# amikey/kaldi-ctc

Measured on AMD Instinct MI355X. Metric: CTC-train frames/sec, 5×BLSTM-512 mb=16, at 1/2/4/8 MI355X; loss match, higher is better.
Workload: dtype f32

## Files before the change

### kaldi-ctc_amd/_bindings.py

```python
import ctypes

vp, ci, cl, cf, cd, sz = (ctypes.c_void_p, ctypes.c_int, ctypes.c_long, ctypes.c_float,
                          ctypes.c_double, ctypes.c_size_t)
ip = ctypes.POINTER(ctypes.c_int)

SIGS = {
    "krnnCreate": (ci, [ctypes.POINTER(vp), ci, ci, ci, ci, ci]),
    "krnnDestroy": (ci, [vp]),
    "krnnGetStatusString": (ctypes.c_char_p, [ci]),
    "krnnGetParamsSize": (sz, [vp]),
    "krnnGetLinLayerOffset": (cl, [vp, ci, ci, ci, ip]),
    "krnnGetWorkspaceSize": (sz, [vp, ci, ci]),
    "krnnGetTrainingReserveSize": (sz, [vp, ci, ci]),
    "krnnForwardTraining": (ci, [vp, vp, ci, ci, vp, vp, vp, vp, sz, vp, sz]),
    "krnnForwardInference": (ci, [vp, vp, ci, ci, vp, vp, vp, vp, sz]),
    "krnnGetInferenceSeqWorkspaceSize": (sz, [vp, ci, ci]),
    "krnnForwardInferenceSeq": (ci, [vp, vp, ci, ci, vp, vp, vp, vp, vp, sz]),
    "krnnBackwardData": (ci, [vp, vp, ci, ci, vp, vp, vp, vp, vp, sz, vp, sz]),
    "krnnBackwardWeights": (ci, [vp, vp, ci, ci, vp, vp, vp, sz, vp, vp, sz]),
    "krnnGetDeviceStatus": (ci, [vp, vp]),
    "kcm_add_mat_mat": (ci, [vp, ci, ci, ci, ci, ci, cf, vp, cl, vp, cl, cf, vp, cl]),
    "kcm_add_mat_mat_x3_workspace": (sz, [ci, ci, ci]),
    "kcm_add_mat_mat_x3": (ci, [vp, ci, ci, ci, ci, ci, cf, vp, cl, vp, cl, cf, vp, cl, vp]),
    "kcm_bench_gemm_packed": (cf, [vp, ci, ci, ci, ci, ci, ci]),
    "kcm_test_gemm_packed": (ci, [vp, ci, ci, ci, ci, ci, ci, ci, ci, vp, vp, vp, vp]),
    "kcm_test_row_stream": (ci, [vp, ci, ci, ci, ci, ci, vp, vp, vp, vp]),
    "kctc_test_component_side_streams": (ci, [vp, ci]),
    "kctc_test_rec6_select": (ci, [ci, ci, ci, ci, ci, ci, ip, ctypes.POINTER(vp)]),
    "kctc_test_rec_plan": (ci, [ci, ci, ci, ci, ci, ci, ctypes.POINTER(cl)]),
    "kcm_find_row_max_id": (ci, [vp, vp, cl, ci, vp]),
    "kcm_clip_gradient_rows": (ci, [vp, vp, cl, ci, cf, vp]),
    "kcm_add_vec_clipped": (ci, [vp, vp, vp, cl, cf, cf]),
    "kcm_add_row_sum_mat": (ci, [vp, vp, cl, ci, cf, cf, vp, vp]),
    "kctc_last_error": (ctypes.c_char_p, []),
    "kctc_nnet_create": (ci, [ctypes.POINTER(vp), ctypes.c_char_p, ctypes.c_ulonglong, ci]),
    "kctc_nnet_destroy": (ci, [vp]),
    "kctc_nnet_num_components": (ci, [vp]),
    "kctc_nnet_context": (ci, [vp, ip, ip]),
    "kctc_nnet_component_info": (ci, [vp, ci, ctypes.c_char_p, sz]),
    "kctc_nnet_num_params": (cl, [vp, ci]),
    "kctc_nnet_get_params": (ci, [vp, ci, vp, cl]),
    "kctc_nnet_set_params": (ci, [vp, ci, vp, cl]),
    "kctc_nnet_get_grad": (ci, [vp, ci, vp, cl]),
    "kctc_nnet_set_learning_rate": (ci, [vp, cf]),
    "kctc_nnet_clip_stats": (ci, [vp, ci, ctypes.POINTER(cd), ctypes.POINTER(cd)]),
    "kctc_nnet_srand": (ci, [vp, ctypes.c_uint]),
    "kctc_nnet_rand_calls": (ci, [vp, ctypes.POINTER(cl)]),
    "kctc_nnet_last_best_path": (ci, [vp, vp, cl]),
    "kctc_nnet_last_output": (ci, [vp, vp, cl]),
    "kctc_nnet_last_costs": (ci, [vp, vp, ci]),
    "kctc_nnet_train_step": (ci, [vp, vp, ci, ci, vp, vp, vp, ctypes.POINTER(cd), ctypes.POINTER(cd),
                                  ctypes.POINTER(cd)]),
# ... 108 lines not shown
```

### kaldi-ctc_amd/csrc/ctc.hip

```cpp
#include <algorithm>
#include <cstring>
#include <type_traits>
#include <atomic>
#include <vector>

#include "common.h"
#include "ctc.h"
#include "prof.h"

namespace kctc {
namespace ctcimpl {

constexpr int kMaxLabel = 639;
constexpr int kThreads = 256;
constexpr int kABThreads = 512;
constexpr int kABWaves = kABThreads / 64;
constexpr int kSPT = (2 * kMaxLabel + 1 + kABThreads - 1) / kABThreads;
constexpr int kFR = 8;

struct UttDesc {
  int T, L, S, feasible, lab_off, pad;
  long long ab_off;
  long long off_off;
};

struct Layout {
  size_t desc, labels, links, owner, costs, logz, lp, spill, offs, total;
  int T_max;
  long long spill_floats, off_doubles;
};
// ... 464 lines not shown

template <bool SPILL>
__global__ __launch_bounds__(64 * kWinWaves) void ctc_alpha_beta_win(
    const float *__restrict__ lp, int N, int A, int blank, UttDesc *__restrict__ descs,
    const int *__restrict__ labels, float *__restrict__ spill, double *__restrict__ offs,
    double *__restrict__ costs, AbLds lay) {
  if (blockIdx.x >= (unsigned)N) win_body<SPILL, true>(lp, N, A, blank, descs, labels, spill, offs, costs, lay);
  else win_body<SPILL, false>(lp, N, A, blank, descs, labels, spill, offs, costs, lay);
}

template <bool SPILL, int SPT>
__global__ __launch_bounds__(kABThreads) void ctc_alpha_beta(
    const float *__restrict__ lp, int N, int A, int blank, UttDesc *__restrict__ descs,
    const int *__restrict__ labels, float *__restrict__ spill, double *__restrict__ offs,
    double *__restrict__ costs, AbLds lay) {
  if (blockIdx.x >= (unsigned)N) ab_body<SPILL, SPT, true>(lp, N, A, blank, descs, labels, spill, offs, costs, lay);
  else ab_body<SPILL, SPT, false>(lp, N, A, blank, descs, labels, spill, offs, costs, lay);
}

__global__ __launch_bounds__(kThreads) void ctc_grad(
    const float *__restrict__ acts, const float *__restrict__ logz, float *__restrict__ grads,
    int N, int A, int T_max, int blank, const UttDesc *__restrict__ descs,
    const int *__restrict__ links, const int *__restrict__ owners, const float *__restrict__ spill,
    const double *__restrict__ offs, const double *__restrict__ costs) {
  extern __shared__ __attribute__((aligned(16))) char smem[];
  const int n = blockIdx.y, t0 = blockIdx.x * kFR, tid = threadIdx.x;
  const UttDesc d = descs[n];
  const int T = d.feasible ? d.T : 0, L = d.L, S = d.S;
  const int nf = min(kFR, T_max - t0);
  if (t0 >= T) {
    for (int it = tid; it < nf * A; it += kThreads) {
      int f = it / A, a = it - f * A;
      grads[((long)(t0 + f) * N + n) * A + a] = 0.f;
    }
    return;
  }
  float *occ = reinterpret_cast<float *>(smem);
  int *nxt = reinterpret_cast<int *>(occ + kFR * S);
  int *owner = nxt + (L > 0 ? L : 1);
  float *gblank = reinterpret_cast<float *>(owner + A);
  float *gtot = gblank + kFR;
  for (int a = tid; a < A; a += kThreads) owner[a] = owners[(long)n * A + a];
  for (int j = tid; j < L; j += kThreads) nxt[j] = links[d.lab_off + j];
  const double logp = -costs[n];
  const float *al = spill + d.ab_off;
  const float *be = al + (long long)T * S;
  const double *oa = offs + d.off_off, *ob = oa + T;
  const int nreal = min(nf, T - t0);
  for (int f = 0; f < nreal; f++) {
    const int t = t0 + f;
    const float Kt = (float)(oa[t] + ob[t] - logp);
    for (int s = tid; s < S; s += kThreads) {
      float v = al[(long)t * S + s] + be[(long)t * S + s];
      occ[f * S + s] = (v == -INFINITY) ? 0.f : expf(v + Kt);
    }
  }
// ... 6 lines not shown
        acc += occ[f * S + s];
        tot += occ[f * S + s] + (s + 1 < S ? occ[f * S + s + 1] : 0.f);
      }
      acc = wave_sum(acc);
      tot = wave_sum(tot);
      if (lane == 0) { gblank[f] = acc / tot; gtot[f] = 1.f / tot; }
    }
  }
  __syncthreads();
  for (int it = tid; it < nf * A; it += kThreads) {
    const int f = it / A, a = it - f * A, t = t0 + f;
    const long idx = ((long)t * N + n) * A + a;
    float g = 0.f;
    if (t < T) {
      float gam = 0.f;
      if (a == blank) {
        gam = gblank[f];
      } else {
        for (int j = owner[a]; j >= 0; j = nxt[j]) gam += occ[f * S + 2 * j + 1];
        gam *= gtot[f];
      }
      g = expf(acts[idx] - logz[(long)t * N + n]) - gam;
    }
    grads[idx] = g;
  }
}

struct Staging {
  char *buf = nullptr;
  size_t cap = 0;
  hipEvent_t ev = nullptr;
  bool pending = false;
};
static thread_local Staging g_stage;

static char *staging_acquire(size_t bytes) {
  Staging &s = g_stage;
  if (s.pending) {
    if (hipEventSynchronize(s.ev) != hipSuccess) return nullptr;
    s.pending = false;
  }
  if (!s.ev && hipEventCreateWithFlags(&s.ev, hipEventDisableTiming) != hipSuccess) return nullptr;
  if (bytes > s.cap) {
    if (s.buf) (void)hipHostFree(s.buf);
    size_t cap = align_up(bytes * 2, 4096);
    if (hipHostMalloc((void **)&s.buf, cap, hipHostMallocDefault) != hipSuccess) {
      s.buf = nullptr; s.cap = 0;
// ... 4 lines not shown
  return s.buf;
}
static void staging_release(hipStream_t stream) {
  if (hipEventRecord(g_stage.ev, stream) == hipSuccess) g_stage.pending = true;
}

static std::atomic<int> g_frame_group{0};
static int frame_group() {
  int m = g_frame_group.load(std::memory_order_relaxed);
  if (m <= 0) {
    m = 8;
    int expect = 0;
    g_frame_group.compare_exchange_strong(expect, m);
    m = g_frame_group.load(std::memory_order_relaxed);
  }
  return m;
}

static std::atomic<int> g_win{1};
static bool win_enabled() { return g_win.load(std::memory_order_relaxed) != 0; }

static ctcStatus_t launch(const float *acts, float *grads, const int *flat_labels,
                          const int *label_lengths, const int *input_lengths, int A, int N,
                          double *costs_dev, void *workspace, hipStream_t stream, int blank) {
  Layout lay;
  std::vector<UttDesc> descs;
  bool bad = false;
  if (!make_layout(label_lengths, input_lengths, A, N, &lay, &descs, &bad) || bad)
    return CTC_STATUS_INVALID_VALUE;
  if (blank < 0 || blank >= A || !acts || !workspace) return CTC_STATUS_INVALID_VALUE;
  long long nlab = 0;
  for (int n = 0; n < N; n++) nlab += label_lengths[n];
  for (long long i = 0; i < nlab; i++)
    if (flat_labels[i] < 0 || flat_labels[i] >= A || flat_labels[i] == blank)
      return CTC_STATUS_INVALID_VALUE;
  char *ws = static_cast<char *>(workspace);
  char *stage = staging_acquire(lay.costs);
  if (!stage) return CTC_STATUS_MEMOPS_FAILED;
  memcpy(stage + lay.desc, descs.data(), sizeof(UttDesc) * N);
  if (nlab) memcpy(stage + lay.labels, flat_labels, sizeof(int) * nlab);
  {
    int *links = reinterpret_cast<int *>(stage + lay.links), *owner = reinterpret_cast<int *>(stage + lay.owner);
    std::fill(owner, owner + (size_t)N * A, -1);
    long long off = 0;
    for (int n = 0; n < N; n++) {
      const int L = label_lengths[n];
      int *own = owner + (size_t)n * A;
// ... 52 lines not shown
        hipLaunchKernelGGL(kern, dim3(grid), dim3(kABThreads), shm, stream, d_lp, N, A, blank, d_desc, d_lab,
                           d_spill, d_offs, costs_dev, al);
      };
      if (Smax <= kABThreads) {
        if (want) go(ctc_alpha_beta<true, 1>, 2 * N);
        else go(ctc_alpha_beta<false, 1>, N);
      } else {
        if (want) go(ctc_alpha_beta<true, kSPT>, 2 * N);
        else go(ctc_alpha_beta<false, kSPT>, N);
      }
    }
  }
  if (want && lay.T_max > 0) {
    int Lmax = 0;
    for (int n = 0; n < N; n++) Lmax = label_lengths[n] > Lmax ? label_lengths[n] : Lmax;
    const int Smax = 2 * Lmax + 1;
    size_t shm = sizeof(float) * kFR * Smax + sizeof(int) * (Lmax > 0 ? Lmax : 1) +
                 sizeof(int) * A + 2 * sizeof(float) * kFR;
    if (shm > 160 * 1024) return CTC_STATUS_INVALID_VALUE;
    ProfSpan ps(stream, "ctc_grad");
    hipLaunchKernelGGL(ctc_grad, dim3(ceil_div(lay.T_max, kFR), N), dim3(kThreads), shm, stream,
                       acts, d_logz, grads, N, A, lay.T_max, blank, d_desc,
                       reinterpret_cast<const int *>(ws + lay.links), reinterpret_cast<const int *>(ws + lay.owner),
                       d_spill, d_offs, costs_dev);
  }
  if (hipGetLastError() != hipSuccess) return CTC_STATUS_EXECUTION_FAILED;
  return CTC_STATUS_SUCCESS;
}

}
}

using namespace kctc::ctcimpl;

extern "C" {

int get_warpctc_version(void) { return 2; }

int mictc_set_frame_group(int m) {
  const int prev = frame_group();
  if (m > 0) g_frame_group.store(std::max(1, std::min(m, 8)));
  return prev;
}

int mictc_set_win(int on) {
  const int prev = g_win.load();
  if (on >= 0) g_win.store(on ? 1 : 0);
// ... 4 lines not shown
  switch (status) {
    case CTC_STATUS_SUCCESS: return "no error";
    case CTC_STATUS_MEMOPS_FAILED: return "cuda memcpy or memset failed";
    case CTC_STATUS_INVALID_VALUE: return "invalid value";
    case CTC_STATUS_EXECUTION_FAILED: return "execution failed";
    case CTC_STATUS_UNKNOWN_ERROR:
    default: return "unknown error";
  }
}

ctcStatus_t get_workspace_size(const int *const label_lengths, const int *const input_lengths,
                               int alphabet_size, int minibatch, struct ctcOptions info,
                               size_t *size_bytes) {
  if (!size_bytes || info.loc != CTC_GPU) return CTC_STATUS_INVALID_VALUE;
  Layout lay;
  bool bad = false;
  if (!make_layout(label_lengths, input_lengths, alphabet_size, minibatch, &lay, nullptr, &bad) ||
      bad)
    return CTC_STATUS_INVALID_VALUE;
  *size_bytes = lay.total;
  return CTC_STATUS_SUCCESS;
}

ctcStatus_t mictc_compute_ctc_loss_async(const float *activations, float *gradients,
                                         const int *flat_labels, const int *label_lengths,
                                         const int *input_lengths, int alphabet_size,
                                         int minibatch, double *costs_dev, void *workspace,
                                         ctcStream_t stream, int blank_label) {
  if (!costs_dev) return CTC_STATUS_INVALID_VALUE;
  try {
    return launch(activations, gradients, flat_labels, label_lengths, input_lengths,
                  alphabet_size, minibatch, costs_dev, workspace,
                  reinterpret_cast<hipStream_t>(stream), blank_label);
  } catch (...) {
    return CTC_STATUS_UNKNOWN_ERROR;
  }
}

ctcStatus_t compute_ctc_loss(const float *const activations, float *gradients,
                             const int *const flat_labels, const int *const label_lengths,
                             const int *const input_lengths, int alphabet_size, int minibatch,
                             float *costs, void *workspace, struct ctcOptions options) {
  if (options.loc != CTC_GPU || !costs) return CTC_STATUS_INVALID_VALUE;
  Layout lay;
  bool bad = false;
  if (!make_layout(label_lengths, input_lengths, alphabet_size, minibatch, &lay, nullptr, &bad) ||
      bad)
    return CTC_STATUS_INVALID_VALUE;
  hipStream_t stream = reinterpret_cast<hipStream_t>(options.stream);
  double *d_costs = reinterpret_cast<double *>(static_cast<char *>(workspace) + lay.costs);
  ctcStatus_t st = mictc_compute_ctc_loss_async(activations, gradients, flat_labels,
                                                label_lengths, input_lengths, alphabet_size,
                                                minibatch, d_costs, workspace, options.stream,
                                                options.blank_label);
  if (st != CTC_STATUS_SUCCESS) return st;
  std::vector<double> hc(minibatch);
  if (hipMemcpyAsync(hc.data(), d_costs, sizeof(double) * minibatch, hipMemcpyDeviceToHost,
                     stream) != hipSuccess)
    return CTC_STATUS_MEMOPS_FAILED;
// ... 7 lines not shown
```

### kaldi-ctc_amd/csrc/elementwise.hip

```cpp
#include "common.h"
#include "elementwise.h"

namespace kctc {
namespace {

typedef float floatx4 __attribute__((ext_vector_type(4)));

__global__ __launch_bounds__(256) void k_clip_sgd(float *__restrict__ w, const float *__restrict__ dw,
                                                  long n, float lr, float clip, const unsigned *skip) {
  if (skip && *skip) return;
  const long n4 = n / 4;
  const long stride = (long)gridDim.x * 256;
  const bool vec = ((uintptr_t)w % 16 == 0) && ((uintptr_t)dw % 16 == 0);
  long i = (long)blockIdx.x * 256 + threadIdx.x;
  if (vec) {
    for (; i < n4; i += stride) {
      floatx4 g = reinterpret_cast<const floatx4 *>(dw)[i];
      floatx4 v = reinterpret_cast<floatx4 *>(w)[i];
#pragma unroll
      for (int j = 0; j < 4; j++) {
        float x = g[j];
        if (clip > 0.f) x = fminf(fmaxf(x, -clip), clip);
        v[j] += lr * x;
      }
// ... 65 lines not shown
      const float x = r[j];
      if (x > v[k]) { v[k] = x; vi[k] = j; }
    }
  }
  if (v[2] > v[0]) { v[0] = v[2]; vi[0] = vi[2]; }
  if (v[3] > v[1]) { v[1] = v[3]; vi[1] = vi[3]; }
  if (v[1] > v[0]) { v[0] = v[1]; vi[0] = vi[1]; }
  float b = v[0];
  int bi = vi[0];
#pragma unroll
  for (int w = 32; w >= 1; w >>= 1) {
    const float ob = __shfl_down(b, w, 64);
    const int oi = __shfl_down(bi, w, 64);
    if (ob > b) { b = ob; bi = oi; }
  }
  if (lane == 0) ids[row] = bi;
}

__global__ __launch_bounds__(256) void k_sum_rows(const float *__restrict__ X, long rows, int cols,
                                                  float alpha, float beta, float *__restrict__ out) {
  __shared__ float part[16][64];
  const int c = blockIdx.x * 64 + (threadIdx.x & 63), g = threadIdx.x >> 6;
  float s = 0.f;
  if (c < cols)
    for (long r = blockIdx.y * 4 + g; r < rows; r += 4L * gridDim.y) s += X[r * cols + c];
  part[g][threadIdx.x & 63] = s;
  __syncthreads();
  if (g == 0 && c < cols) {
    float v = ((part[0][threadIdx.x] + part[1][threadIdx.x]) + part[2][threadIdx.x]) + part[3][threadIdx.x];
    out[(long)blockIdx.y * cols + c] = v;
  }
}

__global__ __launch_bounds__(256) void k_sum_partials(const float *__restrict__ part, int nparts,
                                                      int cols, float alpha, float beta,
                                                      float *__restrict__ out) {
  const int c = blockIdx.x * 256 + threadIdx.x;
  if (c >= cols) return;
  float s = 0.f;
  for (int p = 0; p < nparts; p++) s += part[(long)p * cols + c];
  out[c] = alpha * s + (beta != 0.f ? beta * out[c] : 0.f);
}

__global__ void k_scale(float *p, long n, float a) {
  for (long i = (long)blockIdx.x * 256 + threadIdx.x; i < n; i += (long)gridDim.x * 256) p[i] *= a;
}

__global__ void k_fill(float *p, long n, float v) {
  for (long i = (long)blockIdx.x * 256 + threadIdx.x; i < n; i += (long)gridDim.x * 256) p[i] = v;
}

}

static int grid_for(long n, int per = 256) {
  long b = (n + per - 1) / per;
  return (int)std::max<long>(1, std::min<long>(b, 4096));
}

__global__ __launch_bounds__(256) void k_momentum(float *__restrict__ w, float *__restrict__ delta,
                                                  const float *__restrict__ dw, long n, float lr, float clip,
                                                  float m, const unsigned *skip) {
  if (skip && *skip) return;
  for (long i = (long)blockIdx.x * 256 + threadIdx.x; i < n; i += (long)gridDim.x * 256) {
// ... 232 lines not shown
```

### kaldi-ctc_amd/csrc/gemm.h

```cpp
#pragma once
#include <hip/hip_runtime.h>

namespace kctc {

struct GemmArgs {
  bool transA = false, transB = false;
  int M = 0, N = 0, K = 0;
  float alpha = 1.f, beta = 0.f;
  const float *A = nullptr, *B = nullptr;
  float *C = nullptr;
  long lda = 0, ldb = 0, ldc = 0;
  const float *bias = nullptr, *bias2 = nullptr;
  int batch = 1;
  long strideA = 0, strideB = 0, strideC = 0, strideBias = 0;
  int split_k = 1;
  float *ws = nullptr;
  int max_blocks = 0;
  int *tile_counter = nullptr;
};

void gemm_f32(hipStream_t stream, const GemmArgs &g);
int gemm_pick_split(int M, int N, int K, int batch);

void absmax_f32(hipStream_t stream, const float *X, long ldx, int rows, int cols, unsigned *rmax, unsigned *cmax,
                int batch = 1, long strideX = 0, long strideR = 0, long strideC = 0);

void colsum_f32(hipStream_t stream, const float *X, long ldx, int rows, int cols, float alpha,
                float beta, float *out, int batch = 1, long strideX = 0, long strideOut = 0);

}
```

### kaldi-ctc_amd/csrc/gemm.hip

```cpp
#include "common.h"
#include "gemm.h"

namespace kctc {
namespace {

constexpr int BM = 128, BN = 128, BK = 32, LDK = BK + 4, NT = 256;
constexpr int LDM = BM + 4;
constexpr int OPSZ = (BM * LDK > BK * LDM) ? BM * LDK : BK * LDM;
typedef float floatx4 __attribute__((ext_vector_type(4)));

struct KParams {
  const float *A, *B;
  float *C;
  const float *bias, *bias2;
  long lda, ldb, ldc;
  long strideA, strideB, strideC, strideBias;
  int M, N, K, gx, tiles, batch, split, kchunk;
  float alpha, beta;
  float *ws;
  int vecA, vecB;
  int *counter;
};

template <bool KC>
__device__ __forceinline__ void load_tile(const float *__restrict__ P, long ld, int rows, int r0,
                                          int k0, int kend, int vec, floatx4 (&reg)[4]) {
  const int t = threadIdx.x;
#pragma unroll
  for (int i = 0; i < 4; i++) {
    int r, k;
    if (KC) { r = r0 + (t >> 3) + 32 * i; k = k0 + (t & 7) * 4; }
    else    { k = k0 + (t >> 5) + 8 * i;  r = r0 + (t & 31) * 4; }
    floatx4 v = {0.f, 0.f, 0.f, 0.f};
    if (KC) {
      if (r < rows) {
        const float *p = P + (long)r * ld + k;
        if (vec && k + 3 < kend) {
          v = *reinterpret_cast<const floatx4 *>(p);
        } else {
#pragma unroll
          for (int j = 0; j < 4; j++) v[j] = (k + j < kend) ? p[j] : 0.f;
        }
      }
    } else {
      if (k < kend) {
        const float *p = P + (long)k * ld + r;
        if (vec && r + 3 < rows) {
          v = *reinterpret_cast<const floatx4 *>(p);
        } else {
#pragma unroll
          for (int j = 0; j < 4; j++) v[j] = (r + j < rows) ? p[j] : 0.f;
        }
      }
    }
    reg[i] = v;
  }
}

template <bool KC>
__device__ __forceinline__ void store_tile(float *__restrict__ S, const floatx4 (&reg)[4]) {
  const int t = threadIdx.x;
#pragma unroll
  for (int i = 0; i < 4; i++) {
    if (KC) {
      int r = (t >> 3) + 32 * i, k = (t & 7) * 4;
      *reinterpret_cast<floatx4 *>(S + r * LDK + k) = reg[i];
    } else {
      int k = (t >> 5) + 8 * i, r = (t & 31) * 4;
      *reinterpret_cast<floatx4 *>(S + k * LDM + r) = reg[i];
    }
  }
}

template <bool KC>
__device__ __forceinline__ floatx4 frag(const float *S, int row, int k0) {
  if (KC) return *reinterpret_cast<const floatx4 *>(S + row * LDK + k0);
  return floatx4{S[(k0 + 0) * LDM + row], S[(k0 + 1) * LDM + row], S[(k0 + 2) * LDM + row],
                 S[(k0 + 3) * LDM + row]};
}

template <bool TA, bool TB>
__device__ __forceinline__ void gemm_tile(const KParams &p, float (&lds)[2][2 * OPSZ], int id, int total,
                                          bool remap) {
  const int q = total >> 3, rr = total & 7, xcd = id & 7, loc = id >> 3;
  const int wl = remap ? (xcd < rr ? xcd * (q + 1) : rr * (q + 1) + (xcd - rr) * q) + loc : id;
  const int bz = wl / p.tiles, wg = wl - bz * p.tiles;
  const int tn = wg % p.gx, tm = wg / p.gx;
  const int b = bz % p.batch, ks = bz / p.batch;
  const float *A = p.A + (long)b * p.strideA;
  const float *B = p.B + (long)b * p.strideB;
  const int m0 = tm * BM, n0 = tn * BN;
  const int kbeg = ks * p.kchunk, kend = min(p.K, kbeg + p.kchunk);
  const int lane = threadIdx.x & 63, wid = threadIdx.x >> 6;
  const int wm = (wid >> 1) * 64, wn = (wid & 1) * 64;
  const int fr = lane & 15, fq = lane >> 4;

  const float *Ab = TA ? A + m0 : A + (long)m0 * p.lda;
  const float *Bb = TB ? B + (long)n0 * p.ldb : B + n0;
  const int arows = p.M - m0, brows = p.N - n0;

  floatx4 acc[4][4];
// ... 81 lines not shown
          *c = v;
        }
      }
    }
}

template <bool TA, bool TB>
__global__ __launch_bounds__(NT, 2) void gemm_kernel(KParams p) {
  __shared__ __attribute__((aligned(16))) float lds[2][2 * OPSZ];
  __shared__ int next;
  const int total = p.tiles * p.batch * p.split;
  if (p.counter) {
    while (true) {
      if (threadIdx.x == 0) next = atomicAdd(p.counter, 1);
      __syncthreads();
      const int id = next;
      __syncthreads();
      if (id >= total) break;
      gemm_tile<TA, TB>(p, lds, id, total, false);
    }
    return;
  }
  for (int id = blockIdx.x; id < total; id += gridDim.x) gemm_tile<TA, TB>(p, lds, id, total, true);
}

__global__ __launch_bounds__(256) void absmax_kernel(const float *__restrict__ X, long ldx, int nrows, int ncols,
                                                     long strideX, unsigned *__restrict__ rmax,
                                                     unsigned *__restrict__ cmax, long strideR, long strideC,
                                                     int rows_per_block) {
  const int b = blockIdx.y;
  const float *x = X + (long)b * strideX;
  const int lane = threadIdx.x & 63, w = threadIdx.x >> 6;
  const int r0 = blockIdx.x * rows_per_block, r1 = min(nrows, r0 + rows_per_block);
  __shared__ float cm[4][1024];
  for (int c0 = 0; c0 < ncols; c0 += 1024) {
    float colm[16];
#pragma unroll
    for (int j = 0; j < 16; j++) colm[j] = 0.f;
    for (int r = r0 + w; r < r1; r += 4) {
      float m = 0.f;
#pragma unroll
      for (int j = 0; j < 16; j++) {
        const int c = c0 + j * 64 + lane;
        const float v = c < ncols ? fabsf(x[(long)r * ldx + c]) : 0.f;
        m = fmaxf(m, v);
        colm[j] = fmaxf(colm[j], v);
// ... 48 lines not shown
  if (c < cols)
    for (int r = g; r < rows; r += 4) s += x[(long)r * ldx + c];
  part[g][threadIdx.x & 63] = s;
  __syncthreads();
  if (g == 0 && c < cols) {
    float v = ((part[0][threadIdx.x] + part[1][threadIdx.x]) + part[2][threadIdx.x]) + part[3][threadIdx.x];
    float *o = out + (long)b * strideOut + c;
    *o = alpha * v + (beta != 0.f ? beta * *o : 0.f);
  }
}

}

int gemm_pick_split(int M, int N, int K, int batch) {
  const long tiles = (long)ceil_div(M, BM) * ceil_div(N, BN) * batch;
  if (tiles >= 192 || K < 4 * BK) return 1;
  long want = (256 + tiles - 1) / tiles;
  long maxs = K / (2 * BK);
  if (want > maxs) want = maxs;
  if (want > 64) want = 64;
  return want < 1 ? 1 : (int)want;
}

void gemm_f32(hipStream_t stream, const GemmArgs &g) {
  if (g.M <= 0 || g.N <= 0 || g.batch <= 0) return;
  KParams p;
  p.A = g.A; p.B = g.B; p.C = g.C; p.bias = g.bias; p.bias2 = g.bias2;
  p.lda = g.lda; p.ldb = g.ldb; p.ldc = g.ldc;
  p.strideA = g.strideA; p.strideB = g.strideB; p.strideC = g.strideC; p.strideBias = g.strideBias;
  p.M = g.M; p.N = g.N; p.K = g.K; p.alpha = g.alpha; p.beta = g.beta;
  p.gx = ceil_div(g.N, BN);
  p.tiles = p.gx * ceil_div(g.M, BM);
  p.batch = g.batch;
  p.split = (g.split_k > 1 && g.ws) ? g.split_k : 1;
  p.kchunk = p.split > 1 ? (int)align_up((size_t)ceil_div(g.K, p.split), BK) : (g.K > 0 ? g.K : 1);
  if (p.split > 1) p.split = ceil_div(g.K, p.kchunk);
  p.ws = g.ws;
  auto aligned = [](const void *ptr, long ld, long stride) {
    return ((uintptr_t)ptr % 16 == 0) && (ld % 4 == 0) && (stride % 4 == 0);
  };
  p.vecA = aligned(g.A, g.lda, g.strideA);
  p.vecB = aligned(g.B, g.ldb, g.strideB);
  const int total = p.tiles * p.batch * p.split;
  int blocks = total;
  if (g.max_blocks > 0 && total > g.max_blocks) blocks = std::max(8, g.max_blocks / 8 * 8);
  p.counter = g.tile_counter;
  if (p.counter) KCTC_HIP_CHECK(hipMemsetAsync(p.counter, 0, sizeof(int), stream));
  dim3 grid(blocks);
  if (!g.transA && !g.transB) hipLaunchKernelGGL((gemm_kernel<false, false>), grid, dim3(NT), 0, stream, p);
  else if (!g.transA && g.transB) hipLaunchKernelGGL((gemm_kernel<false, true>), grid, dim3(NT), 0, stream, p);
  else if (g.transA && !g.transB) hipLaunchKernelGGL((gemm_kernel<true, false>), grid, dim3(NT), 0, stream, p);
  else hipLaunchKernelGGL((gemm_kernel<true, true>), grid, dim3(NT), 0, stream, p);
  if (p.split > 1) {
    long total = (long)p.batch * p.M * p.N;
    int blocks = (int)std::min<long>(2048, (total + 255) / 256);
    hipLaunchKernelGGL(splitk_reduce, dim3(blocks), dim3(256), 0, stream, p);
  }
}

void absmax_f32(hipStream_t stream, const float *X, long ldx, int rows, int cols, unsigned *rmax, unsigned *cmax,
                int batch, long strideX, long strideR, long strideC) {
  if (rows <= 0 || cols <= 0 || batch <= 0) return;
  if (cmax) KCTC_HIP_CHECK(hipMemsetAsync(cmax, 0, sizeof(unsigned) * (size_t)(batch > 1 ? strideC * (batch - 1) + cols : cols), stream));
  const int rpb = 64;
  hipLaunchKernelGGL(absmax_kernel, dim3(ceil_div(rows, rpb), batch), dim3(256), 0, stream, X, ldx, rows, cols,
                     strideX, rmax, cmax, strideR, strideC, rpb);
}

void colsum_f32(hipStream_t stream, const float *X, long ldx, int rows, int cols, float alpha,
                float beta, float *out, int batch, long strideX, long strideOut) {
  if (cols <= 0 || batch <= 0) return;
  hipLaunchKernelGGL(colsum_kernel, dim3(ceil_div(cols, 64), batch), dim3(256), 0, stream, X, ldx,
// ... 5 lines not shown
```

### kaldi-ctc_amd/csrc/nnet.cpp

```cpp
#include "nnet.h"
#include "kaldi_io.h"

#include <algorithm>
#include <cmath>
#include <cstdio>
#include <cstring>
#include <iomanip>
#include <iostream>
#include <sstream>

#include "common.h"
#include "ctc.h"
#include "decodable.h"
#include "dropout.h"
#include "elementwise.h"
#include "gemm.h"
#include "prof.h"

namespace kctc {
namespace nnet2 {

int levenshtein(const int *ref, int m, const int *hyp, int n) {
  if (m <= 0) return n > 0 ? n : 0;
  if (n <= 0) return m;
  const int W = (m + 63) / 64;
  int lo = ref[0], hi = ref[0];
  for (int i = 1; i < m; i++) { lo = std::min(lo, ref[i]); hi = std::max(hi, ref[i]); }
  std::vector<uint64_t> peq((size_t)(hi - lo + 2) * W, 0);
  for (int i = 0; i < m; i++) peq[(size_t)(ref[i] - lo) * W + i / 64] |= 1ull << (i % 64);
  std::vector<uint64_t> P(W, ~0ull), M(W, 0ull);
  const uint64_t last = 1ull << ((m - 1) % 64);
  int score = m;
  for (int j = 0; j < n; j++) {
    const int c = hyp[j];
    const uint64_t *eq = &peq[(size_t)((c >= lo && c <= hi) ? c - lo : hi - lo + 1) * W];
// ... 1530 lines not shown
  size_t ws = 0;
  {
    ctcOptions o;
    o.loc = CTC_GPU;
    o.stream = reinterpret_cast<ctcStream_t>(S());
    o.blank_label = 0;
    ctcStatus_t st = get_workspace_size(label_lengths, num_frames, A, N, o, &ws);
    if (st != CTC_STATUS_SUCCESS)
      throw std::runtime_error(std::string("get_workspace_size: ") + ctcGetStatusString(st));
    if (ws > ctc_ws_.bytes) {
      std::vector<int> worst_l(N, std::min(T_max, 639)), worst_t(N, T_max);
      size_t w2 = 0;
      if (get_workspace_size(worst_l.data(), worst_t.data(), A, N, o, &w2) == CTC_STATUS_SUCCESS)
        ws = std::max(ws, w2);
    }
  }
  ctc_ws_.ensure(ws);
  costs_dev_.ensure(sizeof(double) * N);
  ids_dev_.ensure(sizeof(int) * rows);
  CuMatrix &deriv = deriv_a_;
  deriv.Resize(rows, A);
  {
    ProfScope ps("layer_ctc");
    ctcStatus_t st = mictc_compute_ctc_loss_async(out.Data(), update_ ? deriv.Data() : nullptr,
                                                  flat_labels, label_lengths, num_frames, A, N,
                                                  static_cast<double *>(costs_dev_.p), ctc_ws_.p,
                                                  reinterpret_cast<ctcStream_t>(S()), 0);
    if (st != CTC_STATUS_SUCCESS)
      throw std::runtime_error(std::string("compute_ctc_loss: ") + ctcGetStatusString(st));
  }
  {
    ProfScope ps("argmax");
    row_argmax(S(), out.Data(), rows, A, static_cast<int *>(ids_dev_.p));
  }
  if (update_) Backprop(T_max, N);

  Slot &sl = slots_[next_];
  const size_t need = sizeof(double) * N + sizeof(int) * rows + sizeof(unsigned) * C;
  if (need > sl.bytes) {
    if (sl.pinned) {
      if (sl.ev) KCTC_HIP_CHECK(hipEventSynchronize(sl.ev));
      (void)hipHostFree(sl.pinned);
    }
    KCTC_HIP_CHECK(hipHostMalloc((void **)&sl.pinned, need, hipHostMallocDefault));
    sl.bytes = need;
  }
  if (!sl.ev) KCTC_HIP_CHECK(hipEventCreateWithFlags(&sl.ev, hipEventDisableTiming));
  double *hcost = reinterpret_cast<double *>(sl.pinned);
  int *hids = reinterpret_cast<int *>(sl.pinned + sizeof(double) * N);
  unsigned *herr = reinterpret_cast<unsigned *>(hids + rows);
// ... 102 lines not shown
    const CuMatrixBase &in = forward_data_[c];
    CuMatrix &out = forward_data_[c + 1];
    if (comp.IsIdentityForward()) {
      out.SetView(in.Data(), in.NumRows(), comp.OutputDim());
      continue;
    }
    out.Resize((long)T * N, comp.OutputDim());
    const auto *rnn = dynamic_cast<const CuDNNRecurrentComponent *>(&comp);
    const CuDNNRecurrentComponent *next = nullptr;
    if (rnn) {
      int c2 = c + 1;
      while (c2 < C && nnet_->GetComponent(c2).IsIdentityForward()) c2++;
      if (c2 < C) next = dynamic_cast<const CuDNNRecurrentComponent *>(&nnet_->GetComponent(c2));
    }
    if (next) rnn->PropagateChained(in, &out, *next);
    else comp.Propagate(chunk_info_[c], chunk_info_[c + 1], in, &out);
  }
}

void NnetCtcUpdater::Backprop(int T, int N) {
  const int C = nnet_->NumComponents();
  const long rows = (long)T * N;
  const int A = nnet_->OutputDim();
  {
    ProfScope ps("scale");
    scale_inplace(S(), deriv_a_.Data(), rows * (long)A, -1.f);
  }
  CuMatrix *cur = &deriv_a_, *other = &deriv_b_;
  const int first = nnet_->FirstUpdatableComponent();
  int max_dim = A;
  for (int c = 0; c <= C; c++) max_dim = std::max(max_dim, chunk_info_[c].feat_dim);
  std::vector<int> updated;
  for (int c = C - 1; c >= first; c--) {
    Component &comp = nnet_->GetComponent(c);
    const CuMatrixBase &in = forward_data_[c], &outv = forward_data_[c + 1];
    Component *to_update = &comp;
    const bool need_in_deriv = c > first;
    CuMatrixBase *in_deriv = nullptr;
    CuMatrixBase view;
    if (need_in_deriv) {
      if (comp.IsIdentityForward()) {
        view = CuMatrixBase(cur->Data(), rows, comp.InputDim());
        in_deriv = &view;
      } else {
        other->Resize(rows, std::max(comp.InputDim(), max_dim));
        view = CuMatrixBase(other->Data(), rows, comp.InputDim());
        in_deriv = &view;
// ... 36 lines not shown
```

### kaldi-ctc_amd/csrc/nnet.h

```cpp
#pragma once
#include <hip/hip_runtime.h>

#include <cstdint>
#include <iosfwd>
#include <map>
#include <memory>
#include <string>
#include <utility>
#include <vector>

#include "clipgrad.h"
#include "glibc_rand.h"
#include "rnn.h"

namespace kctc {
namespace nnet2 {

struct DevBuf {
  void *p = nullptr;
  size_t bytes = 0;
  DevBuf() = default;
  DevBuf(const DevBuf &) = delete;
  DevBuf &operator=(const DevBuf &) = delete;
  DevBuf(DevBuf &&o) noexcept : p(o.p), bytes(o.bytes) { o.p = nullptr; o.bytes = 0; }
// ... 423 lines not shown
  const CuMatrixBase &ForwardSeq(const float *feats, int T_max, int N, const int *num_frames);
  const std::vector<int> &LastBestPath() const { return last_ids_; }
  const std::vector<double> &LastCosts() const { return last_costs_; }
  const CuMatrixBase &Output() const { return forward_data_.empty() ? empty_ : forward_data_.back(); }
  void Srand(unsigned seed) { repair_rng_.Seed(seed); }
  long RandCalls() const { return repair_rng_.Calls(); }
  void InjectStepError(unsigned word) { inject_err_ = word; }
  void ComponentsChanged();

 private:
  void SetupChunks(int T_max, int N);
  void Propagate(int T, int N);
  void Backprop(int T, int N);
  Nnet *nnet_;
  bool update_;
  GradExchange *exchange_ = nullptr;
  GlibcRand repair_rng_{0};
  std::vector<CuMatrix> forward_data_;
  std::vector<int> last_ids_;
  std::vector<double> last_costs_;
  CuMatrixBase empty_;
  std::vector<ChunkInfo> chunk_info_;
  CuMatrix deriv_a_, deriv_b_;
  DevBuf ctc_ws_, costs_dev_, ids_dev_;
  DevBuf err_word_;
  DevBuf err_flag_;
  unsigned inject_err_ = 0;
  struct Slot {
    char *pinned = nullptr;
    size_t bytes = 0;
    hipEvent_t ev = nullptr;
    int N = 0, nerr = 0;
    long rows = 0;
    std::vector<int> num_frames, labels, label_lengths;
  };
  Slot slots_[2];
  int next_ = 0, pending_ = 0;
};

}
}
```

Baseline: 822,400.

## Add skinny-GEMM kernels, fold CTC grad negation, unroll column-sum reductions

Adds a 64x64-tile MFMA GEMM kernel with an optional deep register-prefetch pipeline, used when M, N or K is at most 64. The aim is better utilisation on the narrow matmuls in the BLSTM. The CTC gradient kernel now applies the sign flip directly, which removes a separate full-matrix scaling pass. The row-sum reduction kernels are unrolled by eight to increase memory-level parallelism. The cost is a large amount of new templated GEMM code with new edge-case handling.

```diff
diff --git a/kaldi-ctc_amd/_bindings.py b/kaldi-ctc_amd/_bindings.py
--- a/kaldi-ctc_amd/_bindings.py
+++ b/kaldi-ctc_amd/_bindings.py
@@ -24,10 +24,12 @@
     "kcm_add_mat_mat_x3": (ci, [vp, ci, ci, ci, ci, ci, cf, vp, cl, vp, cl, cf, vp, cl, vp]),
     "kcm_bench_gemm_packed": (cf, [vp, ci, ci, ci, ci, ci, ci]),
     "kcm_test_gemm_packed": (ci, [vp, ci, ci, ci, ci, ci, ci, ci, ci, vp, vp, vp, vp]),
+    "kcm_test_gemm_f32": (ci, [vp, ci, ci, ci, ci, ci, vp, cl, vp, cl, vp, cl, vp, ci, ci]),
     "kcm_test_row_stream": (ci, [vp, ci, ci, ci, ci, ci, vp, vp, vp, vp]),
     "kctc_test_component_side_streams": (ci, [vp, ci]),
     "kctc_test_rec6_select": (ci, [ci, ci, ci, ci, ci, ci, ip, ctypes.POINTER(vp)]),
     "kctc_test_rec_plan": (ci, [ci, ci, ci, ci, ci, ci, ctypes.POINTER(cl)]),
+    "mictc_compute_ctc_loss_scaled_async": (ci, [vp, vp, vp, vp, vp, ci, ci, vp, vp, vp, ci, cf]),
     "kcm_find_row_max_id": (ci, [vp, vp, cl, ci, vp]),
     "kcm_clip_gradient_rows": (ci, [vp, vp, cl, ci, cf, vp]),
     "kcm_add_vec_clipped": (ci, [vp, vp, vp, cl, cf, cf]),
diff --git a/kaldi-ctc_amd/csrc/ctc.hip b/kaldi-ctc_amd/csrc/ctc.hip
--- a/kaldi-ctc_amd/csrc/ctc.hip
+++ b/kaldi-ctc_amd/csrc/ctc.hip
@@ -6,6 +6,7 @@
 
 #include "common.h"
 #include "ctc.h"
+#include "ctc_internal.h"
 #include "prof.h"
 
 namespace kctc {
@@ -516,7 +517,7 @@
     const float *__restrict__ acts, const float *__restrict__ logz, float *__restrict__ grads,
     int N, int A, int T_max, int blank, const UttDesc *__restrict__ descs,
     const int *__restrict__ links, const int *__restrict__ owners, const float *__restrict__ spill,
-    const double *__restrict__ offs, const double *__restrict__ costs) {
+    const double *__restrict__ offs, const double *__restrict__ costs, float gscale) {
   extern __shared__ __attribute__((aligned(16))) char smem[];
   const int n = blockIdx.y, t0 = blockIdx.x * kFR, tid = threadIdx.x;
   const UttDesc d = descs[n];
@@ -525,7 +526,7 @@
   if (t0 >= T) {
     for (int it = tid; it < nf * A; it += kThreads) {
       int f = it / A, a = it - f * A;
-      grads[((long)(t0 + f) * N + n) * A + a] = 0.f;
+      grads[((long)(t0 + f) * N + n) * A + a] = gscale * 0.f;
     }
     return;
   }
@@ -578,7 +579,7 @@
       }
       g = expf(acts[idx] - logz[(long)t * N + n]) - gam;
     }
-    grads[idx] = g;
+    grads[idx] = gscale * g;
   }
 }
 
@@ -629,7 +630,8 @@
 
 static ctcStatus_t launch(const float *acts, float *grads, const int *flat_labels,
                           const int *label_lengths, const int *input_lengths, int A, int N,
-                          double *costs_dev, void *workspace, hipStream_t stream, int blank) {
+                          double *costs_dev, void *workspace, hipStream_t stream, int blank,
+                          float grad_scale) {
   Layout lay;
   std::vector<UttDesc> descs;
   bool bad = false;
@@ -728,7 +730,7 @@
     hipLaunchKernelGGL(ctc_grad, dim3(ceil_div(lay.T_max, kFR), N), dim3(kThreads), shm, stream,
                        acts, d_logz, grads, N, A, lay.T_max, blank, d_desc,
                        reinterpret_cast<const int *>(ws + lay.links), reinterpret_cast<const int *>(ws + lay.owner),
-                       d_spill, d_offs, costs_dev);
+                       d_spill, d_offs, costs_dev, grad_scale);
   }
   if (hipGetLastError() != hipSuccess) return CTC_STATUS_EXECUTION_FAILED;
   return CTC_STATUS_SUCCESS;
@@ -779,19 +781,29 @@
   return CTC_STATUS_SUCCESS;
 }
 
+ctcStatus_t mictc_compute_ctc_loss_scaled_async(const float *activations, float *gradients,
+                                                const int *flat_labels, const int *label_lengths,
+                                                const int *input_lengths, int alphabet_size,
+                                                int minibatch, double *costs_dev, void *workspace,
+                                                ctcStream_t stream, int blank_label, float grad_scale) {
+  if (!costs_dev || (grad_scale != 1.f && grad_scale != -1.f)) return CTC_STATUS_INVALID_VALUE;
+  try {
+    return launch(activations, gradients, flat_labels, label_lengths, input_lengths,
+                  alphabet_size, minibatch, costs_dev, workspace,
+                  reinterpret_cast<hipStream_t>(stream), blank_label, grad_scale);
+  } catch (...) {
+    return CTC_STATUS_UNKNOWN_ERROR;
+  }
+}
+
 ctcStatus_t mictc_compute_ctc_loss_async(const float *activations, float *gradients,
                                          const int *flat_labels, const int *label_lengths,
                                          const int *input_lengths, int alphabet_size,
                                          int minibatch, double *costs_dev, void *workspace,
                                          ctcStream_t stream, int blank_label) {
-  if (!costs_dev) return CTC_STATUS_INVALID_VALUE;
-  try {
-    return launch(activations, gradients, flat_labels, label_lengths, input_lengths,
-                  alphabet_size, minibatch, costs_dev, workspace,
-                  reinterpret_cast<hipStream_t>(stream), blank_label);
-  } catch (...) {
-    return CTC_STATUS_UNKNOWN_ERROR;
-  }
+  return mictc_compute_ctc_loss_scaled_async(activations, gradients, flat_labels, label_lengths,
+                                             input_lengths, alphabet_size, minibatch, costs_dev,
+                                             workspace, stream, blank_label, 1.f);
 }
 
 ctcStatus_t compute_ctc_loss(const float *const activations, float *gradients,
diff --git a/kaldi-ctc_amd/csrc/ctc_internal.h b/kaldi-ctc_amd/csrc/ctc_internal.h
--- /dev/null
+++ b/kaldi-ctc_amd/csrc/ctc_internal.h
@@ -0,0 +1,14 @@
+#pragma once
+#include "ctc.h"
+
+#ifdef __cplusplus
+extern "C" {
+#endif
+ctcStatus_t mictc_compute_ctc_loss_scaled_async(const float *activations, float *gradients,
+                                                const int *flat_labels, const int *label_lengths,
+                                                const int *input_lengths, int alphabet_size,
+                                                int minibatch, double *costs_dev, void *workspace,
+                                                ctcStream_t stream, int blank_label, float grad_scale);
+#ifdef __cplusplus
+}
+#endif
diff --git a/kaldi-ctc_amd/csrc/elementwise.hip b/kaldi-ctc_amd/csrc/elementwise.hip
--- a/kaldi-ctc_amd/csrc/elementwise.hip
+++ b/kaldi-ctc_amd/csrc/elementwise.hip
@@ -111,8 +111,18 @@
   __shared__ float part[16][64];
   const int c = blockIdx.x * 64 + (threadIdx.x & 63), g = threadIdx.x >> 6;
   float s = 0.f;
-  if (c < cols)
-    for (long r = blockIdx.y * 4 + g; r < rows; r += 4L * gridDim.y) s += X[r * cols + c];
+  if (c < cols) {
+    const long st = 4L * gridDim.y;
+    long r = blockIdx.y * 4 + g;
+    for (; r + 7 * st < rows; r += 8 * st) {
+      float v[8];
+#pragma unroll
+      for (int u = 0; u < 8; u++) v[u] = X[(r + u * st) * cols + c];
+#pragma unroll
+      for (int u = 0; u < 8; u++) s += v[u];
+    }
+    for (; r < rows; r += st) s += X[r * cols + c];
+  }
   part[g][threadIdx.x & 63] = s;
   __syncthreads();
   if (g == 0 && c < cols) {
@@ -127,7 +137,15 @@
   const int c = blockIdx.x * 256 + threadIdx.x;
   if (c >= cols) return;
   float s = 0.f;
-  for (int p = 0; p < nparts; p++) s += part[(long)p * cols + c];
+  int p = 0;
+  for (; p + 7 < nparts; p += 8) {
+    float v[8];
+#pragma unroll
+    for (int u = 0; u < 8; u++) v[u] = part[(long)(p + u) * cols + c];
+#pragma unroll
+    for (int u = 0; u < 8; u++) s += v[u];
+  }
+  for (; p < nparts; p++) s += part[(long)p * cols + c];
   out[c] = alpha * s + (beta != 0.f ? beta * out[c] : 0.f);
 }
 
diff --git a/kaldi-ctc_amd/csrc/gemm.h b/kaldi-ctc_amd/csrc/gemm.h
--- a/kaldi-ctc_amd/csrc/gemm.h
+++ b/kaldi-ctc_amd/csrc/gemm.h
@@ -17,7 +17,11 @@
   float *ws = nullptr;
   int max_blocks = 0;
   int *tile_counter = nullptr;
+  bool generic_tile = false;
 };
+
+enum { kGemmTileGeneric = 0, kGemmTileNarrowN = 1, kGemmTileNarrowM = 2, kGemmTileShortK = 3 };
+int gemm_tile_kind(const GemmArgs &g);
 
 void gemm_f32(hipStream_t stream, const GemmArgs &g);
 int gemm_pick_split(int M, int N, int K, int batch);
diff --git a/kaldi-ctc_amd/csrc/gemm.hip b/kaldi-ctc_amd/csrc/gemm.hip
--- a/kaldi-ctc_amd/csrc/gemm.hip
+++ b/kaldi-ctc_amd/csrc/gemm.hip
@@ -18,19 +18,20 @@
   int M, N, K, gx, tiles, batch, split, kchunk;
   float alpha, beta;
   float *ws;
-  int vecA, vecB;
+  int vecA, vecB, vecC;
   int *counter;
 };
 
-template <bool KC>
+template <bool KC, int ROWS = BM>
 __device__ __forceinline__ void load_tile(const float *__restrict__ P, long ld, int rows, int r0,
-                                          int k0, int kend, int vec, floatx4 (&reg)[4]) {
+                                          int k0, int kend, int vec, floatx4 (&reg)[ROWS / 32]) {
   const int t = threadIdx.x;
-#pragma unroll
-  for (int i = 0; i < 4; i++) {
+  constexpr int TPR = ROWS / 4;
+#pragma unroll
+  for (int i = 0; i < ROWS / 32; i++) {
     int r, k;
     if (KC) { r = r0 + (t >> 3) + 32 * i; k = k0 + (t & 7) * 4; }
-    else    { k = k0 + (t >> 5) + 8 * i;  r = r0 + (t & 31) * 4; }
+    else    { k = k0 + t / TPR + (NT / TPR) * i;  r = r0 + (t % TPR) * 4; }
     floatx4 v = {0.f, 0.f, 0.f, 0.f};
     if (KC) {
       if (r < rows) {
@@ -57,26 +58,69 @@
   }
 }
 
-template <bool KC>
-__device__ __forceinline__ void store_tile(float *__restrict__ S, const floatx4 (&reg)[4]) {
+template <bool KC, int ROWS, bool vec>
+__device__ __forceinline__ void load_tile_raw(const float *__restrict__ P, long ld, int rows, int k0,
+                                              int klast, floatx4 (&reg)[ROWS / 32]) {
   const int t = threadIdx.x;
-#pragma unroll
-  for (int i = 0; i < 4; i++) {
+  constexpr int TPR = ROWS / 4;
+#pragma unroll
+  for (int i = 0; i < ROWS / 32; i++) {
+    int r, k;
+    if (KC) { r = (t >> 3) + 32 * i; k = k0 + (t & 7) * 4; }
+    else    { k = k0 + t / TPR + (NT / TPR) * i;  r = (t % TPR) * 4; }
+    if (vec) {
+      const int rc = min(r, KC ? rows - 1 : rows - 4), kc = min(k, KC ? klast - 3 : klast);
+      reg[i] = *reinterpret_cast<const floatx4 *>(KC ? P + (long)rc * ld + kc : P + (long)kc * ld + rc);
+    } else {
+#pragma unroll
+      for (int j = 0; j < 4; j++) {
+        const int rj = min(KC ? r : r + j, rows - 1), kj = min(KC ? k + j : k, klast);
+        reg[i][j] = P[KC ? (long)rj * ld + kj : (long)kj * ld + rj];
+      }
+    }
+  }
+}
+
+template <bool KC, int ROWS>
+__device__ __forceinline__ void store_tile_z(float *__restrict__ S, const floatx4 (&reg)[ROWS / 32], int rows,
+                                             int k0, int klast) {
+  const int t = threadIdx.x;
+  constexpr int TPR = ROWS / 4, LDR = ROWS + 4;
+#pragma unroll
+  for (int i = 0; i < ROWS / 32; i++) {
+    int r, kl;
+    if (KC) { r = (t >> 3) + 32 * i; kl = (t & 7) * 4; }
+    else    { kl = t / TPR + (NT / TPR) * i;  r = (t % TPR) * 4; }
+    floatx4 v;
+#pragma unroll
+    for (int j = 0; j < 4; j++)
+      v[j] = ((KC ? r : r + j) < rows && k0 + (KC ? kl + j : kl) <= klast) ? reg[i][j] : 0.f;
+    *reinterpret_cast<floatx4 *>(KC ? S + r * LDK + kl : S + kl * LDR + r) = v;
+  }
+}
+
+template <bool KC, int ROWS = BM>
+__device__ __forceinline__ void store_tile(float *__restrict__ S, const floatx4 (&reg)[ROWS / 32]) {
+  const int t = threadIdx.x;
+  constexpr int TPR = ROWS / 4, LDR = ROWS + 4;
+#pragma unroll
+  for (int i = 0; i < ROWS / 32; i++) {
     if (KC) {
       int r = (t >> 3) + 32 * i, k = (t & 7) * 4;
       *reinterpret_cast<floatx4 *>(S + r * LDK + k) = reg[i];
     } else {
-      int k = (t >> 5) + 8 * i, r = (t & 31) * 4;
-      *reinterpret_cast<floatx4 *>(S + k * LDM + r) = reg[i];
-    }
-  }
-}
-
-template <bool KC>
+      int k = t / TPR + (NT / TPR) * i, r = (t % TPR) * 4;
+      *reinterpret_cast<floatx4 *>(S + k * LDR + r) = reg[i];
+    }
+  }
+}
+
+template <bool KC, int ROWS = BM>
 __device__ __forceinline__ floatx4 frag(const float *S, int row, int k0) {
+  constexpr int LDR = ROWS + 4;
   if (KC) return *reinterpret_cast<const floatx4 *>(S + row * LDK + k0);
-  return floatx4{S[(k0 + 0) * LDM + row], S[(k0 + 1) * LDM + row], S[(k0 + 2) * LDM + row],
-                 S[(k0 + 3) * LDM + row]};
+  return floatx4{S[(k0 + 0) * LDR + row], S[(k0 + 1) * LDR + row], S[(k0 + 2) * LDR + row],
+                 S[(k0 + 3) * LDR + row]};
 }
 
 template <bool TA, bool TB>
@@ -204,6 +248,194 @@
     return;
   }
   for (int id = blockIdx.x; id < total; id += gridDim.x) gemm_tile<TA, TB>(p, lds, id, total, true);
+}
+
+constexpr int SB = 64, SLDM = SB + 4, SD = 4;
+constexpr int SOPSZ = (SB * LDK > BK * SLDM) ? SB * LDK : BK * SLDM;
+
+template <bool TA, bool TB, bool WIDE_N, bool DEEP, bool VA, bool VB>
+__global__ __launch_bounds__(NT, DEEP ? 2 : 4) void gemm_skinny_kernel(KParams p) {
+  __shared__ __attribute__((aligned(16))) float lds[2][2 * SOPSZ];
+  constexpr int MI = WIDE_N ? 1 : 4, NJ = WIDE_N ? 4 : 1;
+  const int total = p.tiles * p.batch * p.split, id = blockIdx.x;
+  const int q = total >> 3, rr = total & 7, xcd = id & 7, loc = id >> 3;
+  const int wl = (xcd < rr ? xcd * (q + 1) : rr * (q + 1) + (xcd - rr) * q) + loc;
+  const int bz = wl / p.tiles, wg = wl - bz * p.tiles;
+  const int tn = wg % p.gx, tm = wg / p.gx;
+  const int b = bz % p.batch, ks = bz / p.batch;
+  const float *A = p.A + (long)b * p.strideA;
+  const float *B = p.B + (long)b * p.strideB;
+  const int m0 = tm * SB, n0 = tn * SB;
+  const int kbeg = ks * p.kchunk, kend = min(p.K, kbeg + p.kchunk);
+  const int lane = threadIdx.x & 63, wid = __builtin_amdgcn_readfirstlane(threadIdx.x >> 6);
+  const int wm = WIDE_N ? wid * 16 : 0, wn = WIDE_N ? 0 : wid * 16;
+  const int fr = lane & 15, fq = lane >> 4;
+
+  const float *Ab = TA ? A + m0 : A + (long)m0 * p.lda;
+  const float *Bb = TB ? B + (long)n0 * p.ldb : B + n0;
+  const int arows = p.M - m0, brows = p.N - n0;
+  bool ok[MI][NJ];
+#pragma unroll
+  for (int i = 0; i < MI; i++)
+#pragma unroll
+    for (int j = 0; j < NJ; j++) ok[i][j] = wm + i * 16 < arows && wn + j * 16 < brows;
+
+  floatx4 acc[MI][NJ];
+#pragma unroll
+  for (int i = 0; i < MI; i++)
+#pragma unroll
+    for (int j = 0; j < NJ; j++) acc[i][j] = floatx4{0.f, 0.f, 0.f, 0.f};
+
+  floatx4 ra[DEEP ? SD : 2][2], rb[DEEP ? SD : 2][2];
+  int nk = (kend - kbeg + BK - 1) / BK;
+  if (nk < 0) nk = 0;
+  const int klast = kend - 1;
+  auto load = [&](int slot, int kt) {
+    if constexpr (DEEP) {
+      load_tile_raw<!TA, SB, VA>(Ab, p.lda, arows, kbeg + kt * BK, klast, ra[slot]);
+      load_tile_raw<TB, SB, VB>(Bb, p.ldb, brows, kbeg + kt * BK, klast, rb[slot]);
+    } else {
+      load_tile<!TA, SB>(Ab, p.lda, arows, 0, kbeg + kt * BK, kend, p.vecA, ra[slot]);
+      load_tile<TB, SB>(Bb, p.ldb, brows, 0, kbeg + kt * BK, kend, p.vecB, rb[slot]);
+    }
+  };
+  auto store = [&](int slot, int kt) {
+    if constexpr (DEEP) {
+      store_tile_z<!TA, SB>(lds[kt & 1], ra[slot], arows, kbeg + kt * BK, klast);
+      store_tile_z<TB, SB>(lds[kt & 1] + SOPSZ, rb[slot], brows, kbeg + kt * BK, klast);
+    } else {
+      store_tile<!TA, SB>(lds[kt & 1], ra[slot]);
+      store_tile<TB, SB>(lds[kt & 1] + SOPSZ, rb[slot]);
+    }
+  };
+  auto multiply = [&](int cur, int kleft) {
+    const float *sA = lds[cur], *sB = lds[cur] + SOPSZ;
+#pragma unroll
+    for (int kg = 0; kg < BK / 16; kg++) {
+      if (!DEEP && kg * 16 >= kleft) break;
+      floatx4 fa[MI], fb[NJ];
+#pragma unroll
+      for (int i = 0; i < MI; i++) fa[i] = frag<!TA, SB>(sA, wm + i * 16 + fr, kg * 16 + fq * 4);
+#pragma unroll
+      for (int j = 0; j < NJ; j++) fb[j] = frag<TB, SB>(sB, wn + j * 16 + fr, kg * 16 + fq * 4);
+#pragma unroll
+      for (int i = 0; i < MI; i++)
+#pragma unroll
+        for (int j = 0; j < NJ; j++)
+          if (ok[i][j]) {
+#pragma unroll
+            for (int s = 0; s < 4; s++)
+              acc[i][j] = __builtin_amdgcn_mfma_f32_16x16x4f32(fa[i][s], fb[j][s], acc[i][j], 0, 0, 0);
+          }
+    }
+  };
+  if constexpr (DEEP) {
+#pragma unroll
+    for (int d = 0; d < SD; d++) load(d, d);
+    store(0, 0);
+    __syncthreads();
+    for (int kt0 = 0; kt0 < nk - SD; kt0 += SD) {
+#pragma unroll
+      for (int d = 0; d < SD; d++) {
+        load(d, kt0 + d + SD);
+        multiply(d & 1, BK);
+        store((d + 1) % SD, kt0 + d + 1);
+        __syncthreads();
+      }
+    }
+#pragma unroll
+    for (int d = 0; d < SD; d++) {
+      multiply(d & 1, BK);
+      if (d + 1 < SD) store(d + 1, nk - SD + d + 1);
+      __syncthreads();
+    }
+  } else {
+    if (nk <= 2) {
+      if (nk > 0) load(0, 0);
+      if (nk > 1) load(1, 1);
+      if (nk > 0) store(0, 0);
+      __syncthreads();
+      if (nk > 0) multiply(0, kend - kbeg);
+      if (nk > 1) {
+        store(1, 1);
+        __syncthreads();
+        multiply(1, kend - kbeg - BK);
+      }
+      __syncthreads();
+    } else {
+      load(0, 0);
+      store(0, 0);
+      __syncthreads();
+      for (int kt = 0; kt < nk; kt++) {
+        const bool more = kt + 1 < nk;
+        if (more) load(0, kt + 1);
+        multiply(kt & 1, kend - kbeg - kt * BK);
+        if (more) store(0, kt + 1);
+        __syncthreads();
+      }
+    }
+  }
+
+  if (p.split > 1) {
+    float *W = p.ws + ((long)ks * p.batch + b) * (long)p.M * p.N;
+#pragma unroll
+    for (int i = 0; i < MI; i++)
+#pragma unroll
+      for (int j = 0; j < NJ; j++) {
+        const int col = n0 + wn + j * 16 + fr;
+        if (col >= p.N) continue;
+#pragma unroll
+        for (int r = 0; r < 4; r++) {
+          const int row = m0 + wm + i * 16 + fq * 4 + r;
+          if (row < p.M) W[(long)row * p.N + col] = acc[i][j][r];
+        }
+      }
+    return;
+  }
+  float *C = p.C + (long)b * p.strideC;
+  const float *bias = p.bias ? p.bias + (long)b * p.strideBias : nullptr;
+  const float *bias2 = p.bias2 ? p.bias2 + (long)b * p.strideBias : nullptr;
+  if (WIDE_N && p.vecC && p.beta == 0.f && brows >= SB) {
+    float *T = &lds[0][0] + wid * 16 * SLDM;
+#pragma unroll
+    for (int j = 0; j < NJ; j++) {
+      const int col = n0 + j * 16 + fr;
+      float badd = 0.f;
+      if (bias) badd += bias[col];
+      if (bias2) badd += bias2[col];
+#pragma unroll
+      for (int r = 0; r < 4; r++) T[(fq * 4 + r) * SLDM + j * 16 + fr] = p.alpha * acc[0][j][r] + badd;
+    }
+    __syncthreads();
+#pragma unroll
+    for (int ps = 0; ps < 4; ps++) {
+      const int lr = ps * 4 + fq, row = m0 + wm + lr;
+      if (row < p.M)
+        *reinterpret_cast<floatx4 *>(C + (long)row * p.ldc + n0 + fr * 4) =
+            *reinterpret_cast<const floatx4 *>(T + lr * SLDM + fr * 4);
+    }
+    return;
+  }
+#pragma unroll
+  for (int i = 0; i < MI; i++)
+#pragma unroll
+    for (int j = 0; j < NJ; j++) {
+      const int col = n0 + wn + j * 16 + fr;
+      if (col >= p.N) continue;
+      float badd = 0.f;
+      if (bias) badd += bias[col];
+      if (bias2) badd += bias2[col];
+#pragma unroll
+      for (int r = 0; r < 4; r++) {
+        const int row = m0 + wm + i * 16 + fq * 4 + r;
+        if (row < p.M) {
+          float *c = C + (long)row * p.ldc + col;
+          float v = p.alpha * acc[i][j][r] + badd;
+          if (p.beta != 0.f) v += p.beta * *c;
+          *c = v;
+        }
+      }
+    }
 }
 
 __global__ __launch_bounds__(256) void absmax_kernel(const float *__restrict__ X, long ldx, int nrows, int ncols,
@@ -298,15 +530,27 @@
   return want < 1 ? 1 : (int)want;
 }
 
+int gemm_tile_kind(const GemmArgs &g) {
+  if (g.generic_tile || g.max_blocks > 0 || g.tile_counter) return kGemmTileGeneric;
+  if (const char *e = getenv("KCTC_GEMM_GENERIC"))
+    if (atoi(e)) return kGemmTileGeneric;
+  if (g.N <= SB) return kGemmTileNarrowN;
+  if (g.M <= SB) return kGemmTileNarrowM;
+  if (g.K <= SB) return kGemmTileShortK;
+  return kGemmTileGeneric;
+}
+
 void gemm_f32(hipStream_t stream, const GemmArgs &g) {
   if (g.M <= 0 || g.N <= 0 || g.batch <= 0) return;
+  const int kind = gemm_tile_kind(g);
+  const int bm = kind == kGemmTileGeneric ? BM : SB, bn = kind == kGemmTileGeneric ? BN : SB;
   KParams p;
   p.A = g.A; p.B = g.B; p.C = g.C; p.bias = g.bias; p.bias2 = g.bias2;
   p.lda = g.lda; p.ldb = g.ldb; p.ldc = g.ldc;
   p.strideA = g.strideA; p.strideB = g.strideB; p.strideC = g.strideC; p.strideBias = g.strideBias;
   p.M = g.M; p.N = g.N; p.K = g.K; p.alpha = g.alpha; p.beta = g.beta;
-  p.gx = ceil_div(g.N, BN);
-  p.tiles = p.gx * ceil_div(g.M, BM);
+  p.gx = ceil_div(g.N, bn);
+  p.tiles = p.gx * ceil_div(g.M, bm);
   p.batch = g.batch;
   p.split = (g.split_k > 1 && g.ws) ? g.split_k : 1;
   p.kchunk = p.split > 1 ? (int)align_up((size_t)ceil_div(g.K, p.split), BK) : (g.K > 0 ? g.K : 1);
@@ -317,13 +561,37 @@
   };
   p.vecA = aligned(g.A, g.lda, g.strideA);
   p.vecB = aligned(g.B, g.ldb, g.strideB);
+  p.vecC = aligned(g.C, g.ldc, g.strideC);
   const int total = p.tiles * p.batch * p.split;
   int blocks = total;
   if (g.max_blocks > 0 && total > g.max_blocks) blocks = std::max(8, g.max_blocks / 8 * 8);
   p.counter = g.tile_counter;
   if (p.counter) KCTC_HIP_CHECK(hipMemsetAsync(p.counter, 0, sizeof(int), stream));
   dim3 grid(blocks);
-  if (!g.transA && !g.transB) hipLaunchKernelGGL((gemm_kernel<false, false>), grid, dim3(NT), 0, stream, p);
+  if (kind != kGemmTileGeneric) {
+    const int nk_full = ceil_div(p.kchunk, BK), nk_last = ceil_div(g.K - (p.split - 1) * p.kchunk, BK);
+    const bool deep = g.K > 0 && nk_last % SD == 0 && (p.split == 1 || nk_full % SD == 0);
+    const bool va = p.vecA && (g.transA ? g.M : g.K) % 4 == 0, vb = p.vecB && (g.transB ? g.K : g.N) % 4 == 0;
+#define KCTC_SKINNY3(TA, TB, W)                                                                                    \
+  do {                                                                                                             \
+    if (!deep) hipLaunchKernelGGL((gemm_skinny_kernel<TA, TB, W, false, false, false>), grid, dim3(NT), 0, stream, p); \
+    else if (va && vb) hipLaunchKernelGGL((gemm_skinny_kernel<TA, TB, W, true, true, true>), grid, dim3(NT), 0, stream, p); \
+    else if (va) hipLaunchKernelGGL((gemm_skinny_kernel<TA, TB, W, true, true, false>), grid, dim3(NT), 0, stream, p); \
+    else if (vb) hipLaunchKernelGGL((gemm_skinny_kernel<TA, TB, W, true, false, true>), grid, dim3(NT), 0, stream, p); \
+    else hipLaunchKernelGGL((gemm_skinny_kernel<TA, TB, W, true, false, false>), grid, dim3(NT), 0, stream, p);    \
+  } while (0)
+#define KCTC_SKINNY(TA, TB)                                                                              \
+  do {                                                                                                   \
+    if (kind == kGemmTileNarrowM) KCTC_SKINNY3(TA, TB, false);                                           \
+    else KCTC_SKINNY3(TA, TB, true);                                                                     \
+  } while (0)
+    if (!g.transA && !g.transB) KCTC_SKINNY(false, false);
+    else if (!g.transA && g.transB) KCTC_SKINNY(false, true);
+    else if (g.transA && !g.transB) KCTC_SKINNY(true, false);
+    else KCTC_SKINNY(true, true);
+#undef KCTC_SKINNY3
+#undef KCTC_SKINNY
+  } else if (!g.transA && !g.transB) hipLaunchKernelGGL((gemm_kernel<false, false>), grid, dim3(NT), 0, stream, p);
   else if (!g.transA && g.transB) hipLaunchKernelGGL((gemm_kernel<false, true>), grid, dim3(NT), 0, stream, p);
   else if (g.transA && !g.transB) hipLaunchKernelGGL((gemm_kernel<true, false>), grid, dim3(NT), 0, stream, p);
   else hipLaunchKernelGGL((gemm_kernel<true, true>), grid, dim3(NT), 0, stream, p);
diff --git a/kaldi-ctc_amd/csrc/nnet.cpp b/kaldi-ctc_amd/csrc/nnet.cpp
--- a/kaldi-ctc_amd/csrc/nnet.cpp
+++ b/kaldi-ctc_amd/csrc/nnet.cpp
@@ -4,6 +4,7 @@
 #include <algorithm>
 #include <cmath>
 #include <cstdio>
+#include <cstdlib>
 #include <cstring>
 #include <iomanip>
 #include <iostream>
@@ -11,6 +12,7 @@
 
 #include "common.h"
 #include "ctc.h"
+#include "ctc_internal.h"
 #include "decodable.h"
 #include "dropout.h"
 #include "elementwise.h"
@@ -1587,10 +1589,13 @@
   deriv.Resize(rows, A);
   {
     ProfScope ps("layer_ctc");
-    ctcStatus_t st = mictc_compute_ctc_loss_async(out.Data(), update_ ? deriv.Data() : nullptr,
-                                                  flat_labels, label_lengths, num_frames, A, N,
-                                                  static_cast<double *>(costs_dev_.p), ctc_ws_.p,
-                                                  reinterpret_cast<ctcStream_t>(S()), 0);
+    const char *e = getenv("KCTC_CTC_NEG_GRAD");
+    deriv_negated_ = !(e && atoi(e) == 0);
+    ctcStatus_t st = mictc_compute_ctc_loss_scaled_async(out.Data(), update_ ? deriv.Data() : nullptr,
+                                                         flat_labels, label_lengths, num_frames, A, N,
+                                                         static_cast<double *>(costs_dev_.p), ctc_ws_.p,
+                                                         reinterpret_cast<ctcStream_t>(S()), 0,
+                                                         deriv_negated_ ? -1.f : 1.f);
     if (st != CTC_STATUS_SUCCESS)
       throw std::runtime_error(std::string("compute_ctc_loss: ") + ctcGetStatusString(st));
   }
@@ -1739,7 +1744,7 @@
   const int C = nnet_->NumComponents();
   const long rows = (long)T * N;
   const int A = nnet_->OutputDim();
-  {
+  if (!deriv_negated_) {
     ProfScope ps("scale");
     scale_inplace(S(), deriv_a_.Data(), rows * (long)A, -1.f);
   }
diff --git a/kaldi-ctc_amd/csrc/nnet.h b/kaldi-ctc_amd/csrc/nnet.h
--- a/kaldi-ctc_amd/csrc/nnet.h
+++ b/kaldi-ctc_amd/csrc/nnet.h
@@ -469,6 +469,7 @@
   CuMatrixBase empty_;
   std::vector<ChunkInfo> chunk_info_;
   CuMatrix deriv_a_, deriv_b_;
+  bool deriv_negated_ = false;
   DevBuf ctc_ws_, costs_dev_, ids_dev_;
   DevBuf err_word_;
   DevBuf err_flag_;
```

After: 827,100 (median of 6 runs). About the same (+0.6%).
